# msracver/Relation-Networks-for-Object-Detection

Hardware: AMD Instinct MI355X
Metric: images/sec (1000x600, 300 ROIs) (higher is better)
Workload: dtype bf16; 1 GPU; BASELINE configs[1]: ResNet-101 Faster-RCNN + 2 relation modules (N=300, 16 heads, d=1024) + soft-NMS(0.6) + top-100, 600x1000 images, 300 proposals, random-init weights; launch=hipGraph replay, batches_in_flight=1, parallelism=replicas x1 (no data-path collective), ranks_seen_by_rccl=1

## Files before the change

### relation-networks-for-object-detection_amd/csrc/bottleneck.hip

```cpp
#include "common.h"

namespace relnet {

typedef const __attribute__((address_space(1))) void* gas_ptr;
typedef __attribute__((address_space(3))) void* las_ptr;

__device__ __forceinline__ void chain_glds16(const void* src, unsigned lds_byte_addr) {
  asm volatile("s_mov_b32 m0, %1\n\ts_nop 0\n\tglobal_load_lds_dwordx4 %0, off" ::"v"(src), "s"(lds_byte_addr) : "memory", "m0");
}

struct ChainArgs {
  const unsigned short* m2;
  const unsigned short* x;
  const uint4* w3f;
  const uint4* w1f;
  const float* b3;
  const float* b1;
  const unsigned short* xin;
  const uint4* wpf;
  unsigned short* xn;
  unsigned short* m1;
  int P;
  int H, W, Ho, Wo;
  int dbg;
};

template <int MID, bool STREAM, bool REDUCE = true, int KSPLIT = 1, bool PROJ = false, bool GATHER = false>
__global__ __launch_bounds__(512) void bottleneck_chain_kernel(ChainArgs a) {
  static_assert(!PROJ || (!STREAM && KSPLIT == 1), "the projection form exists for the resident-weight kernel");
  static_assert(!GATHER || (!REDUCE && !PROJ && KSPLIT == 1), "the stride-2 gather exists for the plain expand-only forms");
  static_assert(KSPLIT == 1 || (STREAM && !REDUCE), "k-split passes exist for the streamed expand-only form");
  constexpr int COUT = 4 * MID, KS = MID / 16, KSS = KS / KSPLIT, RT = MID / 32, NP = COUT / 64;
  static_assert(!REDUCE || MID <= 128, "MID = 256 with the second product is chain256_roles_kernel");
  constexpr int W3P = 2 * KSS * 1024, W1P = REDUCE ? 4 * RT * 1024 : 0;
  constexpr int WPP = PROJ ? W3P : 0;
  constexpr int PASSB = W3P + WPP + W1P;
  constexpr int STG = PROJ ? 4096 : 8192;
  constexpr int WBYTES = STREAM ? 2 * PASSB : NP * PASSB;
  extern __shared__ __attribute__((aligned(16))) unsigned char smem[];
  const int tid = threadIdx.x, lane = tid & 63;
  const int wave = __builtin_amdgcn_readfirstlane(tid >> 6);
  const int half = lane >> 5, l31 = lane & 31;
  unsigned char* stage = smem + WBYTES + wave * STG;
  float* sB3 = (float*)(smem + WBYTES + 8 * STG);
  float* sB1 = sB3 + COUT;
  for (int i = tid; i < COUT; i += 512) sB3[i] = a.b3[i];
  if constexpr (REDUCE) for (int i = tid; i < MID; i += 512) sB1[i] = a.b1[i];
  if constexpr (!STREAM) {
    for (int i = tid; i < NP * PASSB / 16; i += 512) {
      const int p = i / (PASSB / 16), r = i % (PASSB / 16);
      uint4 v;
      if (r < W3P / 16) v = a.w3f[(long)p * (W3P / 16) + r];
      else if (r < (W3P + WPP) / 16) v = a.wpf[(long)p * (W3P / 16) + (r - W3P / 16)];
      else { const int q = (r - (W3P + WPP) / 16) >> 6, rt = q >> 2, kk = q & 3; v = a.w1f[((long)rt * (COUT / 16) + p * 4 + kk) * 64 + (r & 63)]; }
      ((uint4*)smem)[i] = v;
    }
  }
  __syncthreads();
  const int ntile = (a.P + 31) / 32;
  const int drow = lane >> 3, dslot = lane & 7;
  unsigned xrow[GATHER ? 4 : 1];
  auto gather_rows = [&](int p0) {
    if constexpr (GATHER) {
      const unsigned hw = (unsigned)(a.Ho * a.Wo);
#pragma unroll
      for (int i = 0; i < 4; ++i) {
        const unsigned q = (unsigned)min(p0 + 8 * i + drow, a.P - 1);
        const unsigned b = q / hw, r = q - b * hw, yo = r / (unsigned)a.Wo, xo = r - yo * (unsigned)a.Wo;
        xrow[i] = ((b * (unsigned)a.H + 2u * yo) * (unsigned)a.W + 2u * xo) * (COUT * 2u);
      }
    }
  };
  auto issue_x = [&](int p0, int p) {
    if constexpr (PROJ) return;
    unsigned char* sb = stage + (p & 1) * 4096;
#pragma unroll
    for (int i = 0; i < 4; ++i) {
      const int row = 8 * i + drow;
      const unsigned off = GATHER ? xrow[i] + (p * 64 + ((dslot ^ ((row >> 1) & 7)) << 3)) * 2u
                                  : ((unsigned)min(p0 + row, a.P - 1) * COUT + p * 64 + ((dslot ^ ((row >> 1) & 7)) << 3)) * 2u;
      __builtin_amdgcn_global_load_lds((gas_ptr)((const unsigned char*)a.x + off), (las_ptr)(sb + i * 1024), 16, 0, 0);
    }
  };
  auto issue_w = [&](int st) {
    if constexpr (STREAM) {
      const int p = st / KSPLIT, kh = st % KSPLIT;
      unsigned char* wb = smem + (st & 1) * PASSB;
#pragma unroll
      for (int i = 0; i < (2 * KSS + (REDUCE ? 4 * RT : 0)) / 8; ++i) {
        const int q = wave + 8 * i;
        if (q < 2 * KSS) {
          const int ct = q / KSS, ks = q % KSS;
          __builtin_amdgcn_global_load_lds((gas_ptr)(a.w3f + ((long)((p * 2 + ct) * KS + kh * KSS + ks) * 64 + lane)), (las_ptr)(wb + q * 1024), 16, 0, 0);
        } else {
          const int q1 = q - 2 * KSS, rt = q1 >> 2, kk = q1 & 3;
          __builtin_amdgcn_global_load_lds((gas_ptr)(a.w1f + ((long)(rt * (COUT / 16) + p * 4 + kk) * 64 + lane)), (las_ptr)(wb + W3P + q1 * 1024), 16, 0, 0);
        }
      }
    }
  };
  auto flush = [&](int p0, int p) {
    const unsigned char* sb = stage + (PROJ ? 0 : (p & 1) * 4096) + lane * 16;
    const uint4 v0 = *(const uint4*)sb, v1 = *(const uint4*)(sb + 1024), v2 = *(const uint4*)(sb + 2048), v3 = *(const uint4*)(sb + 3072);
    asm volatile("s_waitcnt lgkmcnt(0)" ::: "memory");
    auto put = [&](int i, const uint4& v) {
      const int row = 8 * i + drow;
      if (p0 + row < a.P) *(uint4*)((unsigned char*)a.xn + ((unsigned)(p0 + row) * COUT + p * 64 + ((dslot ^ ((row >> 1) & 7)) << 3)) * 2u) = v;
    };
    put(0, v0); put(1, v1); put(2, v2); put(3, v3);
  };

  const int t_first = blockIdx.x * 8 + wave;
  const int t_step = gridDim.x * 8;
  const int n_iter = STREAM ? ((ntile + 7) / 8 - (int)blockIdx.x + (int)gridDim.x - 1) / (int)gridDim.x
                            : (ntile - t_first + t_step - 1) / t_step;
  if (n_iter <= 0) return;
  gather_rows(t_first * 32);
  issue_x(t_first * 32, 0);
  issue_w(0);
  for (int it = 0; it < n_iter; ++it) {
    const int p0 = (t_first + it * t_step) * 32;
    const int px = min(p0 + l31, a.P - 1);
    bf16x8 m2f[KS];
#pragma unroll
    for (int ks = 0; ks < KS; ++ks) m2f[ks] = *(const bf16x8*)(a.m2 + (long)px * MID + 16 * ks + 8 * half);
    bf16x8 xf[PROJ ? KS : 1];
    if constexpr (PROJ) {
#pragma unroll
      for (int ks = 0; ks < KS; ++ks) xf[ks] = *(const bf16x8*)(a.xin + (long)px * MID + 16 * ks + 8 * half);
    }
    f32x16 m1acc[RT];
#pragma unroll
    for (int rt = 0; rt < RT; ++rt)
#pragma unroll
      for (int r = 0; r < 16; ++r) m1acc[rt][r] = 0.f;
#pragma unroll 1
    for (int p = 0; p < NP; ++p) {
      f32x16 acc[2];
#pragma unroll
      for (int kh = 0; kh < KSPLIT; ++kh) {
        const int st = p * KSPLIT + kh;
        if constexpr (STREAM) asm volatile("s_waitcnt vmcnt(0)\n\ts_barrier" ::: "memory");
        else if constexpr (!PROJ) asm volatile("s_waitcnt vmcnt(0)" ::: "memory");
        if (kh == 0) {
          if (!PROJ && p > 0) flush(p0, p - 1);
          if (p + 1 < NP) issue_x(p0, p + 1);
          else if (it + 1 < n_iter) { gather_rows(p0 + t_step * 32); issue_x(p0 + t_step * 32, 0); }
        }
        if (st + 1 < NP * KSPLIT) issue_w(st + 1);
        else if (it + 1 < n_iter) issue_w(0);
        const uint4* w3 = (const uint4*)(smem + (STREAM ? (st & 1) : st) * PASSB);
#pragma unroll
        for (int ct = 0; ct < 2; ++ct) {
          if (kh == 0)
#pragma unroll
            for (int r = 0; r < 16; ++r) acc[ct][r] = 0.f;
#pragma unroll
          for (int ks = 0; ks < KSS; ++ks)
            acc[ct] = __builtin_amdgcn_mfma_f32_32x32x16_bf16(*(const bf16x8*)&w3[(ct * KSS + ks) * 64 + lane], m2f[kh * KSS + ks], acc[ct], 0, 0, 0);
          if constexpr (PROJ) {
            const uint4* wp = (const uint4*)((const unsigned char*)w3 + W3P);
#pragma unroll
            for (int ks = 0; ks < KSS; ++ks)
              acc[ct] = __builtin_amdgcn_mfma_f32_32x32x16_bf16(*(const bf16x8*)&wp[(ct * KSS + ks) * 64 + lane], xf[ks], acc[ct], 0, 0, 0);
          }
        }
      }
      const uint4* w1 = (const uint4*)(smem + (STREAM ? (p & 1) : p) * PASSB + W3P + WPP);
      unsigned char* sb = stage + (PROJ ? 0 : (p & 1) * 4096);
#pragma unroll
      for (int ct = 0; ct < 2; ++ct) {
        uint2 pk[4];
#pragma unroll
        for (int g = 0; g < 4; ++g) {
          uint2* sp = (uint2*)(sb + l31 * 128 + (((ct * 4 + g) ^ ((l31 >> 1) & 7)) << 4) + 8 * half);
          const uint2 xv = PROJ ? make_uint2(0u, 0u) : *sp;
          const float4 bv = *(const float4*)(sB3 + p * 64 + ct * 32 + 8 * g + 4 * half);
          const float v0 = fmaxf(acc[ct][4 * g + 0] + bv.x + bf2f(xv.x & 0xffff), 0.f), v1 = fmaxf(acc[ct][4 * g + 1] + bv.y + bf2f(xv.x >> 16), 0.f);
          const float v2 = fmaxf(acc[ct][4 * g + 2] + bv.z + bf2f(xv.y & 0xffff), 0.f), v3 = fmaxf(acc[ct][4 * g + 3] + bv.w + bf2f(xv.y >> 16), 0.f);
          pk[g] = make_uint2(pack_bf16x2(v0, v1), pack_bf16x2(v2, v3));
          *sp = pk[g];
        }
        if constexpr (REDUCE) {
#pragma unroll
          for (int j = 0; j < 2; ++j) {
            bf16x8 xf;
            *(uint2*)&xf = pk[2 * j];
            *((uint2*)&xf + 1) = pk[2 * j + 1];
#pragma unroll
            for (int rt = 0; rt < RT; ++rt)
              m1acc[rt] = __builtin_amdgcn_mfma_f32_32x32x16_bf16(*(const bf16x8*)&w1[(rt * 4 + ct * 2 + j) * 64 + lane], xf, m1acc[rt], 0, 0, 0);
          }
        }
      }
      asm volatile("s_waitcnt lgkmcnt(0)" ::: "memory");
      __builtin_amdgcn_wave_barrier();
      if constexpr (PROJ) { flush(p0, p); __builtin_amdgcn_wave_barrier(); }
    }
    if constexpr (!PROJ) flush(p0, NP - 1);
    if constexpr (!REDUCE) continue;
    unsigned char* sb = stage + (PROJ ? 0 : ((NP - 1) & 1) * 4096);
#pragma unroll
    for (int hc = 0; hc < RT / 2; ++hc) {
#pragma unroll
      for (int r2 = 0; r2 < 2; ++r2)
#pragma unroll
        for (int g = 0; g < 4; ++g) {
          const int rt = 2 * hc + r2;
          const float4 bv = *(const float4*)(sB1 + rt * 32 + 8 * g + 4 * half);
          const float v0 = fmaxf(m1acc[rt][4 * g + 0] + bv.x, 0.f), v1 = fmaxf(m1acc[rt][4 * g + 1] + bv.y, 0.f);
          const float v2 = fmaxf(m1acc[rt][4 * g + 2] + bv.z, 0.f), v3 = fmaxf(m1acc[rt][4 * g + 3] + bv.w, 0.f);
          *(uint2*)(sb + l31 * 128 + (((r2 * 4 + g) ^ ((l31 >> 1) & 7)) << 4) + 8 * half) = make_uint2(pack_bf16x2(v0, v1), pack_bf16x2(v2, v3));
        }
      asm volatile("s_waitcnt lgkmcnt(0)" ::: "memory");
      __builtin_amdgcn_wave_barrier();
      const unsigned char* sl = sb + lane * 16;
      const uint4 v0 = *(const uint4*)sl, v1 = *(const uint4*)(sl + 1024), v2 = *(const uint4*)(sl + 2048), v3 = *(const uint4*)(sl + 3072);
      asm volatile("s_waitcnt lgkmcnt(0)" ::: "memory");
      auto put = [&](int i, const uint4& v) {
        const int row = 8 * i + drow;
        if (p0 + row < a.P) *(uint4*)(a.m1 + (long)(p0 + row) * MID + hc * 64 + ((dslot ^ ((row >> 1) & 7)) << 3)) = v;
      };
      put(0, v0); put(1, v1); put(2, v2); put(3, v3);
    }
  }
}




constexpr int kRolesLdsBytes = 2 * 32768 + 4 * 4 * 4096 + 4 * 4096 + (1024 + 256) * 4;
__global__ __launch_bounds__(512) void chain256_roles_kernel(ChainArgs a) {
  constexpr int MID = 256, COUT = 4 * MID, KS = MID / 16, RT = MID / 32, NP = COUT / 64, NSTEP = 2 * NP, NTL = 4, NBUF = 4;
  constexpr int W3P = KS * 1024, W1P = 2 * RT * 1024, SLOT = W3P + W1P, WBYTES = 2 * SLOT;
  constexpr int STG = NBUF * 4096, M1S = WBYTES + NTL * STG, BIAS = M1S + NTL * 4096;
  static_assert(BIAS + (COUT + MID) * 4 == kRolesLdsBytes, "host launch and kernel disagree on the LDS layout");
  extern __shared__ __attribute__((aligned(16))) unsigned char smem[];
  const int tid = threadIdx.x, lane = tid & 63;
  const int wave = __builtin_amdgcn_readfirstlane(tid >> 6);
  const int half = lane >> 5, l31 = lane & 31, drow = lane >> 3, dslot = lane & 7;
  const unsigned lds0 = (unsigned)(unsigned long)(las_ptr)smem;
  float* sB3 = (float*)(smem + BIAS);
  float* sB1 = sB3 + COUT;
  for (int i = tid; i < COUT; i += 512) sB3[i] = a.b3[i];
  for (int i = tid; i < MID; i += 512) sB1[i] = a.b1[i];
  const int ntile = (a.P + 31) / 32, nset = (ntile + NTL - 1) / NTL;
  const int n_iter = (nset - (int)blockIdx.x + (int)gridDim.x - 1) / (int)gridDim.x;
  if (n_iter <= 0) return;
  const int G = n_iter * NSTEP, NPASS = n_iter * NP;
  auto tile_p0 = [&](int it, int T) { return (((int)blockIdx.x + it * (int)gridDim.x) * NTL + T) * 32; };
  auto issue_x = [&](int T, int Pg) {
    if (a.dbg & 4) return;
    const int p0 = tile_p0(Pg / NP, T), p = Pg % NP;
    unsigned char* sb = smem + WBYTES + T * STG + (Pg % NBUF) * 4096;
#pragma unroll
    for (int i = 0; i < 4; ++i) {
      const int row = 8 * i + drow;
      const unsigned off = ((unsigned)min(p0 + row, a.P - 1) * COUT + p * 64 + ((dslot ^ ((row >> 1) & 7)) << 3)) * 2u;
      chain_glds16((const unsigned char*)a.x + off, __builtin_amdgcn_readfirstlane(lds0 + (unsigned)(sb - smem) + i * 1024));
    }
  };
  auto issue_w = [&](int g, int l) {
    if (a.dbg & 2) return;
    unsigned char* wb = smem + ((g + 1) & 1) * SLOT;
    const int s3 = (g + 1) % NSTEP, s1 = g % NSTEP;
#pragma unroll
    for (int i = 0; i < 16; ++i) {
      if ((a.dbg & 1) && (i & 1)) continue;
      const int q = l + 2 * i;
      if (q < KS) {
        if (g + 1 < G)
          chain_glds16((const unsigned char*)a.w3f + ((unsigned)((s3 * KS + q) * 1024) + lane * 16u), __builtin_amdgcn_readfirstlane(lds0 + (unsigned)(wb - smem) + q * 1024));
      } else if (g >= 0 && g < G) {
        const int q1 = q - KS, rt = q1 >> 1, j = q1 & 1;
        chain_glds16((const unsigned char*)a.w1f + ((unsigned)((rt * (COUT / 16) + (s1 >> 1) * 4 + (s1 & 1) * 2 + j) * 1024) + lane * 16u), __builtin_amdgcn_readfirstlane(lds0 + (unsigned)(wb - smem) + W3P + q1 * 1024));
      }
    }
  };
  if (wave == 4 || wave == 5) issue_w(-1, wave - 4);
  if (wave >= 6) {
#pragma unroll
    for (int tt = 0; tt < 2; ++tt) { issue_x(2 * (wave - 6) + tt, 0); }
#pragma unroll
    for (int tt = 0; tt < 2; ++tt) { issue_x(2 * (wave - 6) + tt, 1); }
  }
  asm volatile("s_waitcnt vmcnt(0) lgkmcnt(0)\n\ts_barrier" ::: "memory");

  if (wave < 4) {
    const int T = wave;
    unsigned char* const stg = smem + WBYTES + T * STG;
    bf16x8 m2f[KS];
#pragma unroll 1
    for (int g = 0; g <= G + 1; ++g) {
      asm volatile("s_waitcnt lgkmcnt(0)\n\ts_barrier" ::: "memory");
      if (g < G) {
        const int st = g % NSTEP, p = st >> 1, ct = st & 1, Pg = g >> 1;
        if (st == 0) {
          const int px = min(tile_p0(g / NSTEP, T) + l31, a.P - 1);
#pragma unroll
          for (int ks = 0; ks < KS; ++ks) m2f[ks] = *(const bf16x8*)(a.m2 + (long)px * MID + 16 * ks + 8 * half);
          __builtin_amdgcn_s_waitcnt(0x0F70);
        }
        const uint4* w3 = (const uint4*)(smem + (g & 1) * SLOT);
        bf16x8 wf[KS];
#pragma unroll
        for (int ks = 0; ks < KS; ++ks) wf[ks] = *(const bf16x8*)&w3[ks * 64 + lane];
        unsigned char* sb = stg + (Pg % NBUF) * 4096;
        uint2 xv[4];
#pragma unroll
        for (int gq = 0; gq < 4; ++gq) xv[gq] = *(const uint2*)(sb + l31 * 128 + (((ct * 4 + gq) ^ ((l31 >> 1) & 7)) << 4) + 8 * half);
        __builtin_amdgcn_sched_barrier(0);
        f32x16 ac;
#pragma unroll
        for (int r = 0; r < 16; ++r) ac[r] = 0.f;
#pragma unroll
        for (int ks = 0; ks < KS; ++ks)
          ac = __builtin_amdgcn_mfma_f32_32x32x16_bf16(wf[ks], m2f[ks], ac, 0, 0, 0);
#pragma unroll
        for (int gq = 0; gq < 4; ++gq) {
          uint2* sp = (uint2*)(sb + l31 * 128 + (((ct * 4 + gq) ^ ((l31 >> 1) & 7)) << 4) + 8 * half);
          const float4 bv = *(const float4*)(sB3 + p * 64 + ct * 32 + 8 * gq + 4 * half);
          const float v0 = fmaxf(ac[4 * gq + 0] + bv.x + bf2f(xv[gq].x & 0xffff), 0.f), v1 = fmaxf(ac[4 * gq + 1] + bv.y + bf2f(xv[gq].x >> 16), 0.f);
          const float v2 = fmaxf(ac[4 * gq + 2] + bv.z + bf2f(xv[gq].y & 0xffff), 0.f), v3 = fmaxf(ac[4 * gq + 3] + bv.w + bf2f(xv[gq].y >> 16), 0.f);
          *sp = make_uint2(pack_bf16x2(v0, v1), pack_bf16x2(v2, v3));
        }
      }
      if ((g & 1) && g >= 3) {
        const int Pf = (g - 3) >> 1, p0 = tile_p0(Pf / NP, T), p = Pf % NP;
        const unsigned char* sb = stg + (Pf % NBUF) * 4096 + lane * 16;
        const uint4 v0 = *(const uint4*)sb, v1 = *(const uint4*)(sb + 1024), v2 = *(const uint4*)(sb + 2048), v3 = *(const uint4*)(sb + 3072);
        asm volatile("s_waitcnt lgkmcnt(0)" ::: "memory");
        auto put = [&](int i, const uint4& v) {
          const int row = 8 * i + drow;
          if (p0 + row < a.P && !(a.dbg & 8)) *(uint4*)((unsigned char*)a.xn + ((unsigned)(p0 + row) * COUT + p * 64 + ((dslot ^ ((row >> 1) & 7)) << 3)) * 2u) = v;
        };
        put(0, v0); put(1, v1); put(2, v2); put(3, v3);
      }
    }
  } else {
    const int T = wave - 4;
    const unsigned char* const stg = smem + WBYTES + T * STG;
    unsigned char* const m1s = smem + M1S + T * 4096;
    f32x16 m1acc[RT];
#pragma unroll
    for (int rt = 0; rt < RT; ++rt)
#pragma unroll
      for (int r = 0; r < 16; ++r) m1acc[rt][r] = 0.f;
    bool drain = false;
#pragma unroll 1
    for (int g = 0; g <= G + 1; ++g) {
      if (wave < 6) asm volatile("s_waitcnt vmcnt(0)" ::: "memory");
      else if (!(g & 1) && (g >> 1) < NPASS) {
        if (!drain && (g >> 1) + 1 < NPASS) asm volatile("s_waitcnt vmcnt(8)" ::: "memory");
        else asm volatile("s_waitcnt vmcnt(0)" ::: "memory");
        drain = false;
      }
      asm volatile("s_waitcnt lgkmcnt(0)\n\ts_barrier" ::: "memory");
      if (wave < 6) issue_w(g, wave - 4);
      else if (!(g & 1) && (g >> 1) + 2 < NPASS) {
#pragma unroll
        for (int tt = 0; tt < 2; ++tt) issue_x(2 * (wave - 6) + tt, (g >> 1) + 2);
      }
      if (g >= 1 && g <= G) {
        const int h = g - 1, st = h % NSTEP, ct = st & 1, Pg = h >> 1;
        const uint4* w1 = (const uint4*)(smem + (g & 1) * SLOT + W3P);
        const unsigned char* sb = stg + (Pg % NBUF) * 4096;
        bf16x8 xf[2];
#pragma unroll
        for (int j = 0; j < 2; ++j) {
          *(uint2*)&xf[j] = *(const uint2*)(sb + l31 * 128 + (((ct * 4 + 2 * j) ^ ((l31 >> 1) & 7)) << 4) + 8 * half);
          *((uint2*)&xf[j] + 1) = *(const uint2*)(sb + l31 * 128 + (((ct * 4 + 2 * j + 1) ^ ((l31 >> 1) & 7)) << 4) + 8 * half);
        }
        bf16x8 wf[2][RT];
#pragma unroll
        for (int j = 0; j < 2; ++j)
#pragma unroll
          for (int rt = 0; rt < RT; ++rt) wf[j][rt] = *(const bf16x8*)&w1[(rt * 2 + j) * 64 + lane];
        __builtin_amdgcn_sched_barrier(0);
#pragma unroll
        for (int j = 0; j < 2; ++j)
#pragma unroll
          for (int rt = 0; rt < RT; ++rt)
            m1acc[rt] = __builtin_amdgcn_mfma_f32_32x32x16_bf16(wf[j][rt], xf[j], m1acc[rt], 0, 0, 0);
        if (st == NSTEP - 1) {
          const int p0 = tile_p0(h / NSTEP, T);
#pragma unroll
          for (int hc = 0; hc < RT / 2; ++hc) {
#pragma unroll
            for (int r2 = 0; r2 < 2; ++r2)
#pragma unroll
              for (int gq = 0; gq < 4; ++gq) {
                const int rt = 2 * hc + r2;
                const float4 bv = *(const float4*)(sB1 + rt * 32 + 8 * gq + 4 * half);
                const float v0 = fmaxf(m1acc[rt][4 * gq + 0] + bv.x, 0.f), v1 = fmaxf(m1acc[rt][4 * gq + 1] + bv.y, 0.f);
                const float v2 = fmaxf(m1acc[rt][4 * gq + 2] + bv.z, 0.f), v3 = fmaxf(m1acc[rt][4 * gq + 3] + bv.w, 0.f);
                *(uint2*)(m1s + l31 * 128 + (((r2 * 4 + gq) ^ ((l31 >> 1) & 7)) << 4) + 8 * half) = make_uint2(pack_bf16x2(v0, v1), pack_bf16x2(v2, v3));
              }
            asm volatile("s_waitcnt lgkmcnt(0)" ::: "memory");
            __builtin_amdgcn_wave_barrier();
            const unsigned char* sl = m1s + lane * 16;
            const uint4 v0 = *(const uint4*)sl, v1 = *(const uint4*)(sl + 1024), v2 = *(const uint4*)(sl + 2048), v3 = *(const uint4*)(sl + 3072);
            asm volatile("s_waitcnt lgkmcnt(0)" ::: "memory");
            __builtin_amdgcn_wave_barrier();
            auto put = [&](int i, const uint4& v) {
              const int row = 8 * i + drow;
              if (p0 + row < a.P && !(a.dbg & 8)) *(uint4*)(a.m1 + (long)(p0 + row) * MID + hc * 64 + ((dslot ^ ((row >> 1) & 7)) << 3)) = v;
            };
            put(0, v0); put(1, v1); put(2, v2); put(3, v3);
          }
#pragma unroll
          for (int rt = 0; rt < RT; ++rt)
#pragma unroll
            for (int r = 0; r < 16; ++r) m1acc[rt][r] = 0.f;
          drain = true;
        }
      }
    }
  }
}

}

using namespace relnet;

static int g_chain_dbg = 0;
extern "C" void relnet_chain_debug(int flags) { g_chain_dbg = flags; }

extern "C" int relnet_bottleneck_chain(const void* mid2, const void* x, const void* w3f, const void* w1f, const float* b3,
                                       const float* b1, void* x_next, void* mid1_next, long P, int mid, void* stream) {
  RELNET_REQUIRE(mid2 && x && w3f && b3 && x_next, "relnet_bottleneck_chain: null operand");
  RELNET_REQUIRE((w1f && b1 && mid1_next) || (!w1f && !b1 && !mid1_next), "relnet_bottleneck_chain: w1f, b1 and mid1_next are given together (or all NULL: expand + shortcut + ReLU only)");
  RELNET_REQUIRE(mid == 64 || mid == 128 || mid == 256 || (mid == 512 && !mid1_next), "relnet_bottleneck_chain: mid = %d unsupported (64, 128, 256; 512 without the reduce product)", mid);
  RELNET_REQUIRE(P > 0 && P * 8 * mid < (1L << 32), "relnet_bottleneck_chain: bad pixel count %ld (the 4 mid-channel map must stay below 4 GiB)", P);
  ChainArgs a;
  a.m2 = (const unsigned short*)mid2; a.x = (const unsigned short*)x; a.w3f = (const uint4*)w3f; a.w1f = (const uint4*)w1f;
  a.b3 = b3; a.b1 = b1; a.xn = (unsigned short*)x_next; a.m1 = (unsigned short*)mid1_next; a.P = (int)P;
  a.xin = nullptr; a.wpf = nullptr; a.dbg = g_chain_dbg;
  a.H = a.W = a.Ho = a.Wo = 0;
  static relnet::PerDeviceOnce attr_once;
  if (attr_once.first()) {
    hipFuncSetAttribute((const void*)bottleneck_chain_kernel<64, false>, hipFuncAttributeMaxDynamicSharedMemorySize, 160 * 1024);
    hipFuncSetAttribute((const void*)bottleneck_chain_kernel<128, true>, hipFuncAttributeMaxDynamicSharedMemorySize, 160 * 1024);
    hipFuncSetAttribute((const void*)bottleneck_chain_kernel<64, false, false>, hipFuncAttributeMaxDynamicSharedMemorySize, 160 * 1024);
    hipFuncSetAttribute((const void*)bottleneck_chain_kernel<128, true, false>, hipFuncAttributeMaxDynamicSharedMemorySize, 160 * 1024);
    hipFuncSetAttribute((const void*)bottleneck_chain_kernel<256, true, false>, hipFuncAttributeMaxDynamicSharedMemorySize, 160 * 1024);
    hipFuncSetAttribute((const void*)bottleneck_chain_kernel<512, true, false, 2>, hipFuncAttributeMaxDynamicSharedMemorySize, 160 * 1024);
    hipFuncSetAttribute((const void*)chain256_roles_kernel, hipFuncAttributeMaxDynamicSharedMemorySize, 160 * 1024);
  }
  const long ntile = (P + 31) / 32;
  const unsigned grid = (unsigned)(ntile < 8 * 256 ? (ntile + 7) / 8 : 256);
  const size_t lds = 65536  + 65536  + (size_t)5 * mid * 4;
  if (mid1_next) {
    if (mid == 64) bottleneck_chain_kernel<64, false><<<grid, 512, lds, (hipStream_t)stream>>>(a);
    else if (mid == 128) bottleneck_chain_kernel<128, true><<<grid, 512, lds, (hipStream_t)stream>>>(a);
    else {
      const long nset = (ntile + 3) / 4;
      chain256_roles_kernel<<<(unsigned)(nset < 256 ? nset : 256), 512, relnet::kRolesLdsBytes, (hipStream_t)stream>>>(a);
    }
  } else {
    if (mid == 64) bottleneck_chain_kernel<64, false, false><<<grid, 512, lds, (hipStream_t)stream>>>(a);
    else if (mid == 128) bottleneck_chain_kernel<128, true, false><<<grid, 512, lds, (hipStream_t)stream>>>(a);
    else if (mid == 256) bottleneck_chain_kernel<256, true, false><<<grid, 512, lds, (hipStream_t)stream>>>(a);
    else bottleneck_chain_kernel<512, true, false, 2><<<grid, 512, lds, (hipStream_t)stream>>>(a);
  }
  return check_launch("relnet_bottleneck_chain");
}

extern "C" int relnet_bottleneck_chain_s2(const void* mid2, const void* x, const void* w3f, const float* b3, void* x_next, int B,
                                          int H, int W, int mid, void* stream) {
  RELNET_REQUIRE(mid2 && x && w3f && b3 && x_next && x_next != x, "relnet_bottleneck_chain_s2: null operand (or x_next == x: this form is never in place)");
  RELNET_REQUIRE(mid == 64 || mid == 128, "relnet_bottleneck_chain_s2: mid = %d unsupported (64, 128)", mid);
  RELNET_REQUIRE(B > 0 && H > 0 && W > 0 && (long)B * H * W * 8 * mid < (1L << 32),
                 "relnet_bottleneck_chain_s2: bad geometry B=%d H=%d W=%d (the full 4 mid-channel map must stay below 4 GiB)", B, H, W);
  ChainArgs a;
  a.m2 = (const unsigned short*)mid2; a.x = (const unsigned short*)x; a.w3f = (const uint4*)w3f; a.w1f = nullptr;
  a.b3 = b3; a.b1 = nullptr; a.xn = (unsigned short*)x_next; a.m1 = nullptr;
  a.xin = nullptr; a.wpf = nullptr; a.dbg = 0;
  a.H = H; a.W = W; a.Ho = (H - 1) / 2 + 1; a.Wo = (W - 1) / 2 + 1;
  const long P = (long)B * a.Ho * a.Wo;
  a.P = (int)P;
  static relnet::PerDeviceOnce attr_once;
  if (attr_once.first()) {
    hipFuncSetAttribute((const void*)bottleneck_chain_kernel<64, false, false, 1, false, true>, hipFuncAttributeMaxDynamicSharedMemorySize, 160 * 1024);
    hipFuncSetAttribute((const void*)bottleneck_chain_kernel<128, true, false, 1, false, true>, hipFuncAttributeMaxDynamicSharedMemorySize, 160 * 1024);
  }
  const long ntile = (P + 31) / 32;
  const unsigned grid = (unsigned)(ntile < 8 * 256 ? (ntile + 7) / 8 : 256);
  const size_t lds = 65536 + 65536 + (size_t)5 * mid * 4;
  if (mid == 64) bottleneck_chain_kernel<64, false, false, 1, false, true><<<grid, 512, lds, (hipStream_t)stream>>>(a);
  else bottleneck_chain_kernel<128, true, false, 1, false, true><<<grid, 512, lds, (hipStream_t)stream>>>(a);
  return check_launch("relnet_bottleneck_chain_s2");
}

extern "C" int relnet_bottleneck_chain_proj(const void* mid2, const void* x_in, const void* w3f, const void* wpf, const void* w1f,
                                            const float* b3p, const float* b1, void* x_next, void* mid1_next, long P, int mid,
                                            void* stream) {
  RELNET_REQUIRE(mid2 && x_in && w3f && wpf && b3p && x_next, "relnet_bottleneck_chain_proj: null operand");
  RELNET_REQUIRE((w1f && b1 && mid1_next) || (!w1f && !b1 && !mid1_next), "relnet_bottleneck_chain_proj: w1f, b1 and mid1_next are given together (or all NULL)");
  RELNET_REQUIRE(mid == 64, "relnet_bottleneck_chain_proj: mid = %d unsupported (64)", mid);
  RELNET_REQUIRE(P > 0 && P * 8 * mid < (1L << 32), "relnet_bottleneck_chain_proj: bad pixel count %ld (x_next is addressed with 32-bit byte offsets: the 4 mid-channel map must stay below 4 GiB)", P);
  ChainArgs a;
  a.m2 = (const unsigned short*)mid2; a.x = nullptr; a.w3f = (const uint4*)w3f; a.w1f = (const uint4*)w1f;
  a.b3 = b3p; a.b1 = b1; a.xn = (unsigned short*)x_next; a.m1 = (unsigned short*)mid1_next; a.P = (int)P;
  a.xin = (const unsigned short*)x_in; a.wpf = (const uint4*)wpf; a.dbg = 0;
  a.H = a.W = a.Ho = a.Wo = 0;
  static relnet::PerDeviceOnce attr_once;
  if (attr_once.first()) {
    hipFuncSetAttribute((const void*)bottleneck_chain_kernel<64, false, true, 1, true>, hipFuncAttributeMaxDynamicSharedMemorySize, 160 * 1024);
    hipFuncSetAttribute((const void*)bottleneck_chain_kernel<64, false, false, 1, true>, hipFuncAttributeMaxDynamicSharedMemorySize, 160 * 1024);
  }
  const long ntile = (P + 31) / 32;
  const unsigned grid = (unsigned)(ntile < 8 * 256 ? (ntile + 7) / 8 : 256);
  const size_t lds = (size_t)4 * (8192 + 8192 + (mid1_next ? 8192 : 0)) + 8 * 4096 + (size_t)5 * mid * 4;
  if (mid1_next) bottleneck_chain_kernel<64, false, true, 1, true><<<grid, 512, lds, (hipStream_t)stream>>>(a);
  else bottleneck_chain_kernel<64, false, false, 1, true><<<grid, 512, lds, (hipStream_t)stream>>>(a);
  return check_launch("relnet_bottleneck_chain_proj");
}

namespace relnet {

__device__ __attribute__((aligned(16))) const unsigned int g_zero_chunk[4] = {0u, 0u, 0u, 0u};

struct Halo3Args {
  const unsigned short* in;
  const uint4* wf;
  const float* bias;
  unsigned short* out;
  int B, H, W, relu;
  int tiles_x, tiles_y;
  int Ho, Wo;
};

constexpr int kHaloW = 34, kHaloSlots = 40;
constexpr int kHaloBytes = 10 * kHaloSlots * 128;
constexpr int kHalo2Row = 65, kHalo2Even = 33;
constexpr int kHalo2Dma = (9 * kHalo2Row + 7) / 8;
constexpr int kHalo2Bytes = kHalo2Dma * 1024;

template <bool S2>
__global__ __launch_bounds__(512) void conv3x3_c64_halo_kernel(Halo3Args a) {
  constexpr int NR = S2 ? 1 : 2;
  constexpr int HB = S2 ? kHalo2Bytes : kHaloBytes;
  extern __shared__ __attribute__((aligned(16))) unsigned char smem[];
  unsigned char* sOutDense = smem + 2 * HB;
  const int tid = threadIdx.x, lane = tid & 63;
  const int wave = __builtin_amdgcn_readfirstlane(tid >> 6);
  const int half = lane >> 5, l31 = lane & 31;
  const int chh = wave & 1, rg = wave >> 1;
  bf16x8 wfrag[36];
#pragma unroll
  for (int ks = 0; ks < 36; ++ks) wfrag[ks] = *(const bf16x8*)&a.wf[(chh * 36 + ks) * 64 + lane];
  float* sBias = (float*)(smem + 2 * HB + (S2 ? 0 : 32768));
  if (tid < 64) sBias[tid] = a.bias[tid];
  const int per_img = a.tiles_x * a.tiles_y;
  const int ntile = a.B * per_img;

  auto issue_halo = [&](int t, unsigned char* buf) {
    asm volatile("" : "+s"(t));
    const int b = t / per_img, ty = (t % per_img) / a.tiles_x, tx = t % a.tiles_x;
    const int y0 = ty * 8 - 1, x0 = tx * 32 - 1;
    const unsigned short* img = a.in + (long)b * a.H * a.W * 64;
    int ln = lane;
    asm volatile("" : "+v"(ln));
    const int r8 = ln >> 3, slot = ln & 7;
    if constexpr (S2) {
      const int ys = 8 * ty - 1, xs = 64 * tx - 1;
#pragma unroll
      for (int i = 0; i < (kHalo2Dma + 7) / 8; ++i) {
        const int j = wave + 8 * i;
        if (j >= kHalo2Dma) break;
        const int q = 8 * j + r8, hy = q / kHalo2Row, sl = q - kHalo2Row * hy;
        const int hx = sl < kHalo2Even ? 2 * sl : 2 * (sl - kHalo2Even) + 1;
        const int y = ys + hy, x = xs + hx;
        const int sw = (4 * j + (r8 >> 1)) & 7;
        const bool ok = hy < 9 && y >= 0 && y < a.H && x >= 0 && x < a.W;
        const void* src = ok ? (const void*)(img + ((long)y * a.W + x) * 64 + ((slot ^ sw) << 3)) : (const void*)g_zero_chunk;
        __builtin_amdgcn_global_load_lds((gas_ptr)src, (las_ptr)(buf + j * 1024), 16, 0, 0);
      }
      return;
    }
#pragma unroll
    for (int i = 0; i < 7; ++i) {
      const int j = wave + 8 * i;
      if (j >= 50) break;
      const int hy = j / 5, part = j - 5 * hy;
      const int y = y0 + hy, hx = part * 8 + r8, x = x0 + hx;
      const int sw = (4 * (hy + part) + (r8 >> 1)) & 7;
      const bool ok = hx < kHaloW && y >= 0 && y < a.H && x >= 0 && x < a.W;
      const void* src = ok ? (const void*)(img + ((long)y * a.W + x) * 64 + ((slot ^ sw) << 3)) : (const void*)g_zero_chunk;
      __builtin_amdgcn_global_load_lds((gas_ptr)src, (las_ptr)(buf + j * 1024), 16, 0, 0);
    }
  };

  int t = blockIdx.x;
  if (t < ntile) issue_halo(t, smem);
  asm volatile("s_waitcnt vmcnt(0)\n\ts_barrier" ::: "memory");
  int cur = 0;
  for (; t < ntile; t += gridDim.x, cur ^= 1) {
    const int tn = t + gridDim.x;
    if (tn < ntile) issue_halo(tn, smem + (cur ^ 1) * HB);
    const unsigned char* hb = smem + cur * HB;
    unsigned char* sOut = S2 ? smem + cur * HB : sOutDense;
    int lq = l31;
    asm volatile("" : "+v"(lq));
    f32x16 acc[NR];
#pragma unroll
    for (int rr = 0; rr < NR; ++rr)
#pragma unroll
      for (int r = 0; r < 16; ++r) acc[rr][r] = 0.f;
    {
      auto frag = [&](int s_, int rr) -> bf16x8 {
        const int tap = s_ >> 2, kb = s_ & 3, dy = tap / 3, dx = tap % 3;
        const int hp = S2 ? (2 * rg + dy) * kHalo2Row + lq + (dx == 1 ? kHalo2Even : dx >> 1)
                          : (2 * rg + rr + dy) * kHaloSlots + lq + dx;
        return *(const bf16x8*)(hb + hp * 128 + (((2 * kb + half) ^ ((hp >> 1) & 7)) << 4));
      };
      bf16x8 pq[3][NR];
#pragma unroll
      for (int rr = 0; rr < NR; ++rr) { pq[0][rr] = frag(0, rr); pq[1][rr] = frag(1, rr); }
#pragma unroll
      for (int s_ = 0; s_ < 36; ++s_) {
        if (s_ + 2 < 36) {
#pragma unroll
          for (int rr = 0; rr < NR; ++rr) pq[(s_ + 2) % 3][rr] = frag(s_ + 2, rr);
        }
#pragma unroll
        for (int rr = 0; rr < NR; ++rr) acc[rr] = __builtin_amdgcn_mfma_f32_32x32x16_bf16(wfrag[s_], pq[s_ % 3][rr], acc[rr], 0, 0, 0);
        __builtin_amdgcn_sched_barrier(0);
      }
    }
    if constexpr (S2) __builtin_amdgcn_s_barrier();
#pragma unroll
    for (int rr = 0; rr < NR; ++rr) {
      const int p = (NR * rg + rr) * 32 + l31;
#pragma unroll
      for (int g = 0; g < 4; ++g) {
        const float4 bq = *(const float4*)(sBias + chh * 32 + 8 * g + 4 * half);
        float v[4] = {acc[rr][4 * g] + bq.x, acc[rr][4 * g + 1] + bq.y, acc[rr][4 * g + 2] + bq.z, acc[rr][4 * g + 3] + bq.w};
#pragma unroll
        for (int e = 0; e < 4; ++e) v[e] = a.relu ? fmaxf(v[e], 0.f) : v[e];
        *(uint2*)(sOut + p * 128 + (((chh * 4 + g) ^ ((p >> 1) & 7)) << 4) + 8 * half) = make_uint2(pack_bf16x2(v[0], v[1]), pack_bf16x2(v[2], v[3]));
      }
    }
    asm volatile("s_waitcnt lgkmcnt(0)\n\ts_barrier" ::: "memory");
    {
      const int b = t / per_img, ty = (t % per_img) / a.tiles_x, tx = t % a.tiles_x;
      unsigned short* img = a.out + (long)b * a.Ho * a.Wo * 64;
      const unsigned char* so = sOut + wave * (2048 * NR) + lane * 16;
      const uint4 v0 = *(const uint4*)so, v1 = *(const uint4*)(so + 1024);
      uint4 v2 = v0, v3 = v1;
      if constexpr (NR == 2) { v2 = *(const uint4*)(so + 2048); v3 = *(const uint4*)(so + 3072); }
      asm volatile("s_waitcnt vmcnt(0) lgkmcnt(0)" ::: "memory");
      auto put = [&](int i, const uint4& v) {
        const int p = 8 * (wave * 2 * NR + i) + (lane >> 3), slot = lane & 7;
        const int y = ty * 4 * NR + (p >> 5), x = tx * 32 + (p & 31);
        if (y < a.Ho && x < a.Wo) *(uint4*)(img + ((long)y * a.Wo + x) * 64 + ((slot ^ ((p >> 1) & 7)) << 3)) = v;
      };
      put(0, v0); put(1, v1);
      if constexpr (NR == 2) { put(2, v2); put(3, v3); }
    }
    __builtin_amdgcn_s_barrier();
  }
}

}

extern "C" int relnet_conv3x3_c64(const void* in, const void* w_frag, const float* bias, int relu, void* out, int B, int H,
                                  int W, void* stream) {
  RELNET_REQUIRE(in && w_frag && bias && out, "relnet_conv3x3_c64: null operand");
  RELNET_REQUIRE(B > 0 && H > 0 && W > 0 && (long)B * H * W < (1L << 31), "relnet_conv3x3_c64: bad geometry B=%d H=%d W=%d", B, H, W);
  Halo3Args a;
  a.in = (const unsigned short*)in; a.wf = (const uint4*)w_frag; a.bias = bias; a.out = (unsigned short*)out;
  a.B = B; a.H = H; a.W = W; a.relu = relu;
  a.tiles_x = (W + 31) / 32; a.tiles_y = (H + 7) / 8; a.Ho = H; a.Wo = W;
  static relnet::PerDeviceOnce attr_once;
  if (attr_once.first()) {
    hipFuncSetAttribute((const void*)conv3x3_c64_halo_kernel<false>, hipFuncAttributeMaxDynamicSharedMemorySize, 160 * 1024);
  }
  const long ntile = (long)B * a.tiles_x * a.tiles_y;
  const unsigned grid = (unsigned)(ntile < 256 ? ntile : 256);
  conv3x3_c64_halo_kernel<false><<<grid, 512, 2 * kHaloBytes + 32768 + 256, (hipStream_t)stream>>>(a);
  return check_launch("relnet_conv3x3_c64");
}

extern "C" int relnet_conv3x3_c64_s2(const void* in, const void* w_frag, const float* bias, int relu, void* out, int B, int H,
                                     int W, void* stream) {
  RELNET_REQUIRE(in && w_frag && bias && out, "relnet_conv3x3_c64_s2: null operand");
  RELNET_REQUIRE(B > 0 && H > 0 && W > 0 && (long)B * H * W < (1L << 31), "relnet_conv3x3_c64_s2: bad geometry B=%d H=%d W=%d", B, H, W);
  Halo3Args a;
  a.in = (const unsigned short*)in; a.wf = (const uint4*)w_frag; a.bias = bias; a.out = (unsigned short*)out;
  a.B = B; a.H = H; a.W = W; a.relu = relu;
  a.Ho = (H - 1) / 2 + 1; a.Wo = (W - 1) / 2 + 1;
  a.tiles_x = (a.Wo + 31) / 32; a.tiles_y = (a.Ho + 3) / 4;
  static relnet::PerDeviceOnce attr_once;
  if (attr_once.first()) {
    hipFuncSetAttribute((const void*)conv3x3_c64_halo_kernel<true>, hipFuncAttributeMaxDynamicSharedMemorySize, 160 * 1024);
  }
  const long ntile = (long)B * a.tiles_x * a.tiles_y;
  const unsigned grid = (unsigned)(ntile < 256 ? ntile : 256);
  conv3x3_c64_halo_kernel<true><<<grid, 512, 2 * kHalo2Bytes + 256, (hipStream_t)stream>>>(a);
  return check_launch("relnet_conv3x3_c64_s2");
}
```

Baseline: 2998 images/s.

## Restructure chain256 roles kernel: full-width expand passes, per-wave w1 register streaming

Each expand wave now processes both 32-channel halves of a 64-channel pass in one step, halving the barrier-separated steps, with double-buffered LDS weight fragment reads interleaved with MFMAs and raised wave priority. Producer waves no longer stage the reduce (w1) weights in LDS. Each of the four producer waves instead owns a 64-channel slice of the reduce output across all four tiles and streams its w1 fragments straight into registers with global loads and counted vmcnt waits, while all four waves share the w3 and x LDS staging. This cuts LDS traffic and barrier count and widens MFMA reuse of each weight fragment across tiles. It relies on hand-tuned vmcnt counts and s_nop padding, adds register pressure from 8 accumulators per wave, and fragile waitcnt accounting could break correctness.

Result: faster. 3037 images/s, median of 6 (+1.3%).

```diff
diff --git a/relation-networks-for-object-detection_amd/csrc/bottleneck.hip b/relation-networks-for-object-detection_amd/csrc/bottleneck.hip
--- a/relation-networks-for-object-detection_amd/csrc/bottleneck.hip
+++ b/relation-networks-for-object-detection_amd/csrc/bottleneck.hip
@@ -229,10 +229,15 @@
 
 
 
+__device__ __forceinline__ void chain_gld16(bf16x8& d, const void* sbase, unsigned voff) {
+  asm volatile("s_nop 4\n\tglobal_load_dwordx4 %0, %1, %2" : "=v"(d) : "v"(voff), "s"(sbase) : "memory");
+}
+__device__ __forceinline__ void chain_wait_frag(bf16x8& d) { asm volatile("s_waitcnt vmcnt(19)" : "+v"(d) : : "memory"); }
+
 constexpr int kRolesLdsBytes = 2 * 32768 + 4 * 4 * 4096 + 4 * 4096 + (1024 + 256) * 4;
 __global__ __launch_bounds__(512) void chain256_roles_kernel(ChainArgs a) {
-  constexpr int MID = 256, COUT = 4 * MID, KS = MID / 16, RT = MID / 32, NP = COUT / 64, NSTEP = 2 * NP, NTL = 4, NBUF = 4;
-  constexpr int W3P = KS * 1024, W1P = 2 * RT * 1024, SLOT = W3P + W1P, WBYTES = 2 * SLOT;
+  constexpr int MID = 256, COUT = 4 * MID, KS = MID / 16, NP = COUT / 64, NTL = 4, NBUF = 4;
+  constexpr int SLOT = 2 * KS * 1024, WBYTES = 2 * SLOT;
   constexpr int STG = NBUF * 4096, M1S = WBYTES + NTL * STG, BIAS = M1S + NTL * 4096;
   static_assert(BIAS + (COUT + MID) * 4 == kRolesLdsBytes, "host launch and kernel disagree on the LDS layout");
   extern __shared__ __attribute__((aligned(16))) unsigned char smem[];
@@ -247,7 +252,7 @@
   const int ntile = (a.P + 31) / 32, nset = (ntile + NTL - 1) / NTL;
   const int n_iter = (nset - (int)blockIdx.x + (int)gridDim.x - 1) / (int)gridDim.x;
   if (n_iter <= 0) return;
-  const int G = n_iter * NSTEP, NPASS = n_iter * NP;
+  const int G = n_iter * NP;
   auto tile_p0 = [&](int it, int T) { return (((int)blockIdx.x + it * (int)gridDim.x) * NTL + T) * 32; };
   auto issue_x = [&](int T, int Pg) {
     if (a.dbg & 4) return;
@@ -260,24 +265,18 @@
       chain_glds16((const unsigned char*)a.x + off, __builtin_amdgcn_readfirstlane(lds0 + (unsigned)(sb - smem) + i * 1024));
     }
   };
-  auto issue_w = [&](int g, int l) {
+  auto issue_w3 = [&](int g, int b) {
     if (a.dbg & 2) return;
-    unsigned char* wb = smem + ((g + 1) & 1) * SLOT;
-    const int s3 = (g + 1) % NSTEP, s1 = g % NSTEP;
-#pragma unroll
-    for (int i = 0; i < 16; ++i) {
-      if ((a.dbg & 1) && (i & 1)) continue;
-      const int q = l + 2 * i;
-      if (q < KS) {
-        if (g + 1 < G)
-          chain_glds16((const unsigned char*)a.w3f + ((unsigned)((s3 * KS + q) * 1024) + lane * 16u), __builtin_amdgcn_readfirstlane(lds0 + (unsigned)(wb - smem) + q * 1024));
-      } else if (g >= 0 && g < G) {
-        const int q1 = q - KS, rt = q1 >> 1, j = q1 & 1;
-        chain_glds16((const unsigned char*)a.w1f + ((unsigned)((rt * (COUT / 16) + (s1 >> 1) * 4 + (s1 & 1) * 2 + j) * 1024) + lane * 16u), __builtin_amdgcn_readfirstlane(lds0 + (unsigned)(wb - smem) + W3P + q1 * 1024));
-      }
+    const int first = b < 2 ? 12 * b : 16 + 4 * b, n = b < 2 ? 12 : 4;
+    const unsigned lb = lds0 + (unsigned)(((g + 1) & 1) * SLOT);
+    const unsigned char* src = (const unsigned char*)a.w3f + (unsigned)(((g + 1) % NP) * SLOT) + lane * 16u;
+#pragma unroll
+    for (int i = 0; i < 12; ++i) {
+      if (i >= n || ((a.dbg & 1) && (i & 1))) continue;
+      chain_glds16(src + (first + i) * 1024, __builtin_amdgcn_readfirstlane(lb + (unsigned)((first + i) * 1024)));
     }
   };
-  if (wave == 4 || wave == 5) issue_w(-1, wave - 4);
+  if (wave >= 4) issue_w3(-1, wave - 4);
   if (wave >= 6) {
 #pragma unroll
     for (int tt = 0; tt < 2; ++tt) { issue_x(2 * (wave - 6) + tt, 0); }
@@ -290,43 +289,66 @@
     const int T = wave;
     unsigned char* const stg = smem + WBYTES + T * STG;
     bf16x8 m2f[KS];
+    __builtin_amdgcn_s_setprio(2);
 #pragma unroll 1
-    for (int g = 0; g <= G + 1; ++g) {
+    for (int g = 0; g <= G; ++g) {
       asm volatile("s_waitcnt lgkmcnt(0)\n\ts_barrier" ::: "memory");
       if (g < G) {
-        const int st = g % NSTEP, p = st >> 1, ct = st & 1, Pg = g >> 1;
-        if (st == 0) {
-          const int px = min(tile_p0(g / NSTEP, T) + l31, a.P - 1);
+        const int p = g % NP;
+        if (p == 0) {
+          const int px = min(tile_p0(g / NP, T) + l31, a.P - 1);
 #pragma unroll
           for (int ks = 0; ks < KS; ++ks) m2f[ks] = *(const bf16x8*)(a.m2 + (long)px * MID + 16 * ks + 8 * half);
           __builtin_amdgcn_s_waitcnt(0x0F70);
         }
         const uint4* w3 = (const uint4*)(smem + (g & 1) * SLOT);
-        bf16x8 wf[KS];
-#pragma unroll
-        for (int ks = 0; ks < KS; ++ks) wf[ks] = *(const bf16x8*)&w3[ks * 64 + lane];
-        unsigned char* sb = stg + (Pg % NBUF) * 4096;
-        uint2 xv[4];
-#pragma unroll
-        for (int gq = 0; gq < 4; ++gq) xv[gq] = *(const uint2*)(sb + l31 * 128 + (((ct * 4 + gq) ^ ((l31 >> 1) & 7)) << 4) + 8 * half);
+        unsigned char* sb = stg + (g % NBUF) * 4096;
+        uint2 xv[2][4];
+#pragma unroll
+        for (int ct = 0; ct < 2; ++ct)
+#pragma unroll
+          for (int gq = 0; gq < 4; ++gq) xv[ct][gq] = *(const uint2*)(sb + l31 * 128 + (((ct * 4 + gq) ^ ((l31 >> 1) & 7)) << 4) + 8 * half);
+        f32x16 ac[2];
+#pragma unroll
+        for (int ct = 0; ct < 2; ++ct)
+#pragma unroll
+          for (int r = 0; r < 16; ++r) ac[ct][r] = 0.f;
+        bf16x8 wf[2][8];
+        auto read_w3 = [&](int set, int bt) {
+#pragma unroll
+          for (int i = 0; i < 4; ++i)
+#pragma unroll
+            for (int ct = 0; ct < 2; ++ct) wf[set][2 * i + ct] = *(const bf16x8*)&w3[(ct * KS + 4 * bt + i) * 64 + lane];
+        };
+        read_w3(0, 0);
+        read_w3(1, 1);
         __builtin_amdgcn_sched_barrier(0);
-        f32x16 ac;
-#pragma unroll
-        for (int r = 0; r < 16; ++r) ac[r] = 0.f;
-#pragma unroll
-        for (int ks = 0; ks < KS; ++ks)
-          ac = __builtin_amdgcn_mfma_f32_32x32x16_bf16(wf[ks], m2f[ks], ac, 0, 0, 0);
-#pragma unroll
-        for (int gq = 0; gq < 4; ++gq) {
-          uint2* sp = (uint2*)(sb + l31 * 128 + (((ct * 4 + gq) ^ ((l31 >> 1) & 7)) << 4) + 8 * half);
-          const float4 bv = *(const float4*)(sB3 + p * 64 + ct * 32 + 8 * gq + 4 * half);
-          const float v0 = fmaxf(ac[4 * gq + 0] + bv.x + bf2f(xv[gq].x & 0xffff), 0.f), v1 = fmaxf(ac[4 * gq + 1] + bv.y + bf2f(xv[gq].x >> 16), 0.f);
-          const float v2 = fmaxf(ac[4 * gq + 2] + bv.z + bf2f(xv[gq].y & 0xffff), 0.f), v3 = fmaxf(ac[4 * gq + 3] + bv.w + bf2f(xv[gq].y >> 16), 0.f);
-          *sp = make_uint2(pack_bf16x2(v0, v1), pack_bf16x2(v2, v3));
-        }
-      }
-      if ((g & 1) && g >= 3) {
-        const int Pf = (g - 3) >> 1, p0 = tile_p0(Pf / NP, T), p = Pf % NP;
+#pragma unroll
+        for (int bt = 0; bt < 4; ++bt) {
+#pragma unroll
+          for (int i = 0; i < 4; ++i)
+#pragma unroll
+            for (int ct = 0; ct < 2; ++ct) ac[ct] = __builtin_amdgcn_mfma_f32_32x32x16_bf16(wf[bt & 1][2 * i + ct], m2f[4 * bt + i], ac[ct], 0, 0, 0);
+          __builtin_amdgcn_sched_barrier(0);
+          if (bt + 2 < 4) {
+            read_w3(bt & 1, bt + 2);
+            __builtin_amdgcn_sched_barrier(0);
+          }
+        }
+#pragma unroll
+        for (int ct = 0; ct < 2; ++ct)
+#pragma unroll
+          for (int gq = 0; gq < 4; ++gq) {
+            uint2* sp = (uint2*)(sb + l31 * 128 + (((ct * 4 + gq) ^ ((l31 >> 1) & 7)) << 4) + 8 * half);
+            const float4 bv = *(const float4*)(sB3 + p * 64 + ct * 32 + 8 * gq + 4 * half);
+            const uint2 x2 = xv[ct][gq];
+            const float v0 = fmaxf(ac[ct][4 * gq + 0] + bv.x + bf2f(x2.x & 0xffff), 0.f), v1 = fmaxf(ac[ct][4 * gq + 1] + bv.y + bf2f(x2.x >> 16), 0.f);
+            const float v2 = fmaxf(ac[ct][4 * gq + 2] + bv.z + bf2f(x2.y & 0xffff), 0.f), v3 = fmaxf(ac[ct][4 * gq + 3] + bv.w + bf2f(x2.y >> 16), 0.f);
+            *sp = make_uint2(pack_bf16x2(v0, v1), pack_bf16x2(v2, v3));
+          }
+      }
+      if (g >= 1) {
+        const int Pf = g - 1, p0 = tile_p0(Pf / NP, T), p = Pf % NP;
         const unsigned char* sb = stg + (Pf % NBUF) * 4096 + lane * 16;
         const uint4 v0 = *(const uint4*)sb, v1 = *(const uint4*)(sb + 1024), v2 = *(const uint4*)(sb + 2048), v3 = *(const uint4*)(sb + 3072);
         asm volatile("s_waitcnt lgkmcnt(0)" ::: "memory");
@@ -338,84 +360,117 @@
       }
     }
   } else {
-    const int T = wave - 4;
-    const unsigned char* const stg = smem + WBYTES + T * STG;
-    unsigned char* const m1s = smem + M1S + T * 4096;
-    f32x16 m1acc[RT];
-#pragma unroll
-    for (int rt = 0; rt < RT; ++rt)
-#pragma unroll
-      for (int r = 0; r < 16; ++r) m1acc[rt][r] = 0.f;
+    const int b = wave - 4;
+    unsigned char* const m1s = smem + M1S + b * 4096;
+    const unsigned lrd = (unsigned)(l31 * 128 + 8 * half) | (unsigned)(((l31 >> 1) & 7) << 4);
+    const unsigned voff = lane * 16u;
+    f32x16 m1acc[NTL][2];
+#pragma unroll
+    for (int T = 0; T < NTL; ++T)
+#pragma unroll
+      for (int r2 = 0; r2 < 2; ++r2)
+#pragma unroll
+        for (int r = 0; r < 16; ++r) m1acc[T][r2][r] = 0.f;
+    bf16x8 wf[8];
+#pragma unroll
+    for (int j = 0; j < 8; ++j) wf[j] = bf16x8{0, 0, 0, 0, 0, 0, 0, 0};
+    auto load_w1 = [&](int j, int pass) {
+      if ((a.dbg & 2) || ((a.dbg & 1) && (j & 1))) return;
+      chain_gld16(wf[j], (const unsigned char*)a.w1f + (unsigned)((((2 * b + (j & 1)) * (COUT / 16)) + 4 * pass + (j >> 1)) * 1024), voff);
+    };
     bool drain = false;
+    asm volatile("s_waitcnt lgkmcnt(0)\n\ts_barrier" ::: "memory");
+    issue_w3(0, b);
+    if (wave >= 6) {
+#pragma unroll
+      for (int tt = 0; tt < 2; ++tt) issue_x(2 * (wave - 6) + tt, 2);
+    }
+#pragma unroll
+    for (int j = 0; j < 8; ++j) load_w1(j, 0);
 #pragma unroll 1
-    for (int g = 0; g <= G + 1; ++g) {
-      if (wave < 6) asm volatile("s_waitcnt vmcnt(0)" ::: "memory");
-      else if (!(g & 1) && (g >> 1) < NPASS) {
-        if (!drain && (g >> 1) + 1 < NPASS) asm volatile("s_waitcnt vmcnt(8)" ::: "memory");
-        else asm volatile("s_waitcnt vmcnt(0)" ::: "memory");
-        drain = false;
-      }
+    for (int g = 1; g <= G; ++g) {
+      if (drain) asm volatile("s_waitcnt vmcnt(0)" ::: "memory");
+      else if (wave < 6) asm volatile("s_waitcnt vmcnt(8)" ::: "memory");
+      else asm volatile("s_waitcnt vmcnt(16)" ::: "memory");
+      drain = false;
       asm volatile("s_waitcnt lgkmcnt(0)\n\ts_barrier" ::: "memory");
-      if (wave < 6) issue_w(g, wave - 4);
-      else if (!(g & 1) && (g >> 1) + 2 < NPASS) {
-#pragma unroll
-        for (int tt = 0; tt < 2; ++tt) issue_x(2 * (wave - 6) + tt, (g >> 1) + 2);
-      }
-      if (g >= 1 && g <= G) {
-        const int h = g - 1, st = h % NSTEP, ct = st & 1, Pg = h >> 1;
-        const uint4* w1 = (const uint4*)(smem + (g & 1) * SLOT + W3P);
-        const unsigned char* sb = stg + (Pg % NBUF) * 4096;
-        bf16x8 xf[2];
-#pragma unroll
-        for (int j = 0; j < 2; ++j) {
-          *(uint2*)&xf[j] = *(const uint2*)(sb + l31 * 128 + (((ct * 4 + 2 * j) ^ ((l31 >> 1) & 7)) << 4) + 8 * half);
-          *((uint2*)&xf[j] + 1) = *(const uint2*)(sb + l31 * 128 + (((ct * 4 + 2 * j + 1) ^ ((l31 >> 1) & 7)) << 4) + 8 * half);
-        }
-        bf16x8 wf[2][RT];
-#pragma unroll
-        for (int j = 0; j < 2; ++j)
-#pragma unroll
-          for (int rt = 0; rt < RT; ++rt) wf[j][rt] = *(const bf16x8*)&w1[(rt * 2 + j) * 64 + lane];
+      const int q = g - 1, p = q % NP, pn = g % NP;
+      const unsigned char* sb = smem + WBYTES + (q % NBUF) * 4096;
+      uint2 xr[NTL][2];
+      bf16x8 xf[NTL];
+      unsigned tb[NTL];
+#pragma unroll
+      for (int T = 0; T < NTL; ++T) { tb[T] = (unsigned)(T * STG); asm volatile("" : "+v"(tb[T])); }
+      auto read_x = [&](int kk) {
+#pragma unroll
+        for (int T = 0; T < NTL; ++T) {
+          xr[T][0] = *(const uint2*)(sb + tb[T] + (lrd ^ (unsigned)((2 * kk) << 4)));
+          xr[T][1] = *(const uint2*)(sb + tb[T] + (lrd ^ (unsigned)((2 * kk + 1) << 4)));
+        }
+      };
+      auto join_x = [&]() {
+#pragma unroll
+        for (int T = 0; T < NTL; ++T) { *(uint2*)&xf[T] = xr[T][0]; *((uint2*)&xf[T] + 1) = xr[T][1]; }
+      };
+      read_x(0);
+      __builtin_amdgcn_sched_barrier(0);
+      issue_w3(g, b);
+      if (wave >= 6) {
+#pragma unroll
+        for (int tt = 0; tt < 2; ++tt) issue_x(2 * (wave - 6) + tt, g + 2);
+      }
+      join_x();
+#pragma unroll
+      for (int kk = 0; kk < 4; ++kk) {
         __builtin_amdgcn_sched_barrier(0);
-#pragma unroll
-        for (int j = 0; j < 2; ++j)
-#pragma unroll
-          for (int rt = 0; rt < RT; ++rt)
-            m1acc[rt] = __builtin_amdgcn_mfma_f32_32x32x16_bf16(wf[j][rt], xf[j], m1acc[rt], 0, 0, 0);
-        if (st == NSTEP - 1) {
-          const int p0 = tile_p0(h / NSTEP, T);
-#pragma unroll
-          for (int hc = 0; hc < RT / 2; ++hc) {
-#pragma unroll
-            for (int r2 = 0; r2 < 2; ++r2)
-#pragma unroll
-              for (int gq = 0; gq < 4; ++gq) {
-                const int rt = 2 * hc + r2;
-                const float4 bv = *(const float4*)(sB1 + rt * 32 + 8 * gq + 4 * half);
-                const float v0 = fmaxf(m1acc[rt][4 * gq + 0] + bv.x, 0.f), v1 = fmaxf(m1acc[rt][4 * gq + 1] + bv.y, 0.f);
-                const float v2 = fmaxf(m1acc[rt][4 * gq + 2] + bv.z, 0.f), v3 = fmaxf(m1acc[rt][4 * gq + 3] + bv.w, 0.f);
-                *(uint2*)(m1s + l31 * 128 + (((r2 * 4 + gq) ^ ((l31 >> 1) & 7)) << 4) + 8 * half) = make_uint2(pack_bf16x2(v0, v1), pack_bf16x2(v2, v3));
-              }
-            asm volatile("s_waitcnt lgkmcnt(0)" ::: "memory");
-            __builtin_amdgcn_wave_barrier();
-            const unsigned char* sl = m1s + lane * 16;
-            const uint4 v0 = *(const uint4*)sl, v1 = *(const uint4*)(sl + 1024), v2 = *(const uint4*)(sl + 2048), v3 = *(const uint4*)(sl + 3072);
-            asm volatile("s_waitcnt lgkmcnt(0)" ::: "memory");
-            __builtin_amdgcn_wave_barrier();
-            auto put = [&](int i, const uint4& v) {
-              const int row = 8 * i + drow;
-              if (p0 + row < a.P && !(a.dbg & 8)) *(uint4*)(a.m1 + (long)(p0 + row) * MID + hc * 64 + ((dslot ^ ((row >> 1) & 7)) << 3)) = v;
-            };
-            put(0, v0); put(1, v1); put(2, v2); put(3, v3);
-          }
-#pragma unroll
-          for (int rt = 0; rt < RT; ++rt)
-#pragma unroll
-            for (int r = 0; r < 16; ++r) m1acc[rt][r] = 0.f;
-          drain = true;
-        }
-      }
-    }
+        if (kk + 1 < 4) {
+          read_x(kk + 1);
+          __builtin_amdgcn_sched_barrier(0);
+        }
+#pragma unroll
+        for (int r2 = 0; r2 < 2; ++r2) {
+          const int j = 2 * kk + r2;
+          chain_wait_frag(wf[j]);
+#pragma unroll
+          for (int T = 0; T < NTL; ++T) m1acc[T][r2] = __builtin_amdgcn_mfma_f32_32x32x16_bf16(wf[j], xf[T], m1acc[T][r2], 0, 0, 0);
+          __builtin_amdgcn_sched_barrier(0);
+          load_w1(j, pn);
+        }
+        if (kk + 1 < 4) join_x();
+      }
+      if (p == NP - 1) {
+#pragma unroll
+        for (int T = 0; T < NTL; ++T) {
+          const int p0 = tile_p0(q / NP, T);
+#pragma unroll
+          for (int r2 = 0; r2 < 2; ++r2)
+#pragma unroll
+            for (int gq = 0; gq < 4; ++gq) {
+              const float4 bv = *(const float4*)(sB1 + (2 * b + r2) * 32 + 8 * gq + 4 * half);
+              const float v0 = fmaxf(m1acc[T][r2][4 * gq + 0] + bv.x, 0.f), v1 = fmaxf(m1acc[T][r2][4 * gq + 1] + bv.y, 0.f);
+              const float v2 = fmaxf(m1acc[T][r2][4 * gq + 2] + bv.z, 0.f), v3 = fmaxf(m1acc[T][r2][4 * gq + 3] + bv.w, 0.f);
+              *(uint2*)(m1s + l31 * 128 + (((r2 * 4 + gq) ^ ((l31 >> 1) & 7)) << 4) + 8 * half) = make_uint2(pack_bf16x2(v0, v1), pack_bf16x2(v2, v3));
+            }
+          asm volatile("s_waitcnt lgkmcnt(0)" ::: "memory");
+          __builtin_amdgcn_wave_barrier();
+          const unsigned char* sl = m1s + lane * 16;
+          const uint4 v0 = *(const uint4*)sl, v1 = *(const uint4*)(sl + 1024), v2 = *(const uint4*)(sl + 2048), v3 = *(const uint4*)(sl + 3072);
+          asm volatile("s_waitcnt lgkmcnt(0)" ::: "memory");
+          __builtin_amdgcn_wave_barrier();
+          auto put = [&](int i, const uint4& v) {
+            const int row = 8 * i + drow;
+            if (p0 + row < a.P && !(a.dbg & 8)) *(uint4*)(a.m1 + (long)(p0 + row) * MID + b * 64 + ((dslot ^ ((row >> 1) & 7)) << 3)) = v;
+          };
+          put(0, v0); put(1, v1); put(2, v2); put(3, v3);
+#pragma unroll
+          for (int r2 = 0; r2 < 2; ++r2)
+#pragma unroll
+            for (int r = 0; r < 16; ++r) m1acc[T][r2][r] = 0.f;
+        }
+        drain = true;
+      }
+    }
+    asm volatile("s_waitcnt vmcnt(0)" ::: "memory");
   }
 }
 
```
